# BUTSpeechFIT/TS-ASR-Whisper

Measured on AMD Instinct MI355X. Metric: train utterances/sec (30 s clips) whisper-large-v3-turbo DiCoW, higher is better.
Workload: dtype bf16; 1 GPU; whisper-large-v3-turbo DiCoW fine-tune step, per-GPU batch 16, L=128, decoder frozen, bf16 AMP; global_batch=16, parallelism=dp1, split_streams=False, trainable_params=637306880

## Files before the change

ts-asr-whisper_amd/csrc/gemm.hip:

```cpp
#include <stdlib.h>
#include "common.h"

#define BM 128
#define BN 128
#define BK 64
#define STAGE_BYTES (BM * BK * 2)
#define NT_LDS_BYTES (4 * STAGE_BYTES)
#define NT_FDDT_FLAGS (DICOW_EPI_BIAS | DICOW_EPI_RESIDUAL | DICOW_EPI_OUT_F32 | DICOW_EPI_FDDT)
#define NT_RES_FLAGS (DICOW_EPI_BIAS | DICOW_EPI_RESIDUAL | DICOW_EPI_OUT_F32)
#define NT_RES_LN_FLAGS (NT_RES_FLAGS | DICOW_EPI_LNSTAT)
#define NT_FDDT_LN_FLAGS (NT_FDDT_FLAGS | DICOW_EPI_LNSTAT)
#define NT_QKV_LN_FLAGS (DICOW_EPI_BIAS | DICOW_EPI_SCALE_N | DICOW_EPI_LNFOLD)
#define NT_FC1I_LN_FLAGS (DICOW_EPI_BIAS | DICOW_EPI_GELU | DICOW_EPI_LNFOLD)
#define NT_FC1T_LN_FLAGS (DICOW_EPI_BIAS | DICOW_EPI_GELU | DICOW_EPI_GELU_DAUX | DICOW_EPI_LNFOLD)

typedef __attribute__((address_space(3))) void lds_void_t;
typedef const __attribute__((address_space(1))) void gbl_void_t;

__device__ __forceinline__ void glds16(const void* gsrc, void* lds_dst) {
    __builtin_amdgcn_global_load_lds((gbl_void_t*)gsrc, (lds_void_t*)lds_dst, 16, 0, 0);
}

#ifndef NT_GM
#define NT_GM 8
// ... 507 lines not shown
__device__ __forceinline__ float ln_dpp(float old, float x) {
    return __int_as_float(__builtin_amdgcn_update_dpp(__float_as_int(old), __float_as_int(x), CTRL, 0xf, BANK, false));
}
template <int CTRL>
__device__ __forceinline__ float ln_merge(float a, float b, bool bit) {
    const float keep = bit ? b : a, send = bit ? a : b;
    return keep + ln_dpp<CTRL>(0.f, send);
}
__device__ __forceinline__ float ln_xor4(float x) { return ln_dpp<0x114, 0xA>(ln_dpp<0x104, 0x5>(0.f, x), x); }
__device__ __forceinline__ float ln_merge4(float a, float b, bool bit) {
    const float keep = bit ? b : a, send = bit ? a : b;
    return keep + ln_xor4(send);
}
#include "gemm_ntr.inc"
#ifndef NT2_MASK
#define NT2_MASK 0
#endif
#ifndef NT2_SLOTS
#define NT2_SLOTS 2
#endif
#ifndef NT2_DELAY
#define NT2_DELAY 0
#endif
#ifndef NTQ_MASK
#define NTQ_MASK 0
#endif
#if defined(DICOW_EXPERIMENTS) || defined(DICOW_ABLATIONS) || NT2_MASK || NTQ_MASK
#define NT_EXPERIMENT_KERNELS 1
#include "experiments/gemm_nt2.inc"
#include "experiments/gemm_ntq.inc"
#else
#define NT_EXPERIMENT_KERNELS 0
#endif

#ifdef DICOW_ABLATIONS
#include "experiments/gemm_nt256s.inc"
#endif

#include <atomic>
#include <mutex>
static std::atomic<int> g_gemm_cus{0};
extern "C" int dicow_set_gemm_cus(int n) { return g_gemm_cus.exchange(n > 0 ? n : 0); }

#include <map>
#include <mutex>
#include <string>
static std::mutex g_disp_mu;
static std::map<std::string, long> g_disp;
static void disp_note(const char* fmt, int a0 = 0, int a1 = 0, int a2 = 0) {
    char b[96];
    snprintf(b, sizeof b, fmt, a0, a1, a2);
    std::lock_guard<std::mutex> lk(g_disp_mu);
    ++g_disp[b];
}
extern "C" int dicow_gemm_dispatch_log(char* buf, int cap) {
    std::lock_guard<std::mutex> lk(g_disp_mu);
    int n = 0;
    for (const auto& kv : g_disp) {
        const int w = snprintf(buf ? buf + n : nullptr, buf && cap > n ? cap - n : 0, "%s\t%ld\n", kv.first.c_str(), kv.second);
        if (w < 0) break;
        n += w;
        if (buf && n >= cap) { n = cap - 1; break; }
    }
    return n;
}

#ifndef NT_BIG_TILES
#define NT_BIG_TILES 200
#endif
#ifndef NT64_MAX_TILES128
#define NT64_MAX_TILES128 128
#endif

#define NT_EPILOGUES_COMMON(X)                                                                                                  \
    X(0) X(DICOW_EPI_BIAS) X(DICOW_EPI_BIAS | DICOW_EPI_SCALE_N) X(DICOW_EPI_BIAS | DICOW_EPI_GELU) X(NT_RES_FLAGS)             \
    X(DICOW_EPI_BIAS | DICOW_EPI_GELU | DICOW_EPI_GELU_DAUX) X(DICOW_EPI_MUL_AUX) X(DICOW_EPI_MUL_AUX | DICOW_EPI_COLSUM)
#ifdef DICOW_EXPERIMENTS
#define NT_HAS_LN_EPILOGUES 1
#define NT_EPILOGUES_LN(BOTH, W35) W35(NT_RES_LN_FLAGS) W35(NT_FDDT_LN_FLAGS) BOTH(NT_QKV_LN_FLAGS) BOTH(NT_FC1I_LN_FLAGS) BOTH(NT_FC1T_LN_FLAGS)
#else
#define NT_HAS_LN_EPILOGUES 0
#define NT_EPILOGUES_LN(BOTH, W35)
#endif
#define NT_EPILOGUES(BOTH, W35) BOTH(-1) NT_EPILOGUES_COMMON(BOTH) W35(NT_FDDT_FLAGS) NT_EPILOGUES_LN(BOTH, W35)

static int g_ncu_all = 256;
static int nt_ncu() {
    const int lim = g_gemm_cus.load();
    return (lim > 0 && lim < g_ncu_all) ? lim : g_ncu_all;
}

static void gemm_nt_setup() {
    (void)hipFuncSetAttribute((const void*)gemm_nt_kernel<2, false>, hipFuncAttributeMaxDynamicSharedMemorySize, NT_LDS_BYTES);
    (void)hipFuncSetAttribute((const void*)gemm_nt128t_kernel, hipFuncAttributeMaxDynamicSharedMemorySize, NT_LDS_BYTES);
    (void)hipFuncSetAttribute((const void*)gemm_nt64_kernel<8>, hipFuncAttributeMaxDynamicSharedMemorySize, 8 * 16384);
    (void)hipFuncSetAttribute((const void*)gemm_nt64_kernel<4>, hipFuncAttributeMaxDynamicSharedMemorySize, 4 * 16384);
    (void)hipFuncSetAttribute((const void*)gemm_nt_kernel<2, true>, hipFuncAttributeMaxDynamicSharedMemorySize, NT_LDS_BYTES);
#define W35(F) (void)hipFuncSetAttribute((const void*)gemm_ntr_kernel<(F), 3, 5>, hipFuncAttributeMaxDynamicSharedMemorySize, NTR_LDS);
#define BOTH(F) (void)hipFuncSetAttribute((const void*)gemm_ntr_kernel<(F), 4, 4>, hipFuncAttributeMaxDynamicSharedMemorySize, NTR_LDS); W35(F)
    NT_EPILOGUES(BOTH, W35)
#undef BOTH
#undef W35
    hipDeviceProp_t pr;
    int dev = 0;
    (void)hipGetDevice(&dev);
    if (hipGetDeviceProperties(&pr, dev) == hipSuccess) g_ncu_all = pr.multiProcessorCount;
}

static int nt_ct_flags(int flags) {
    switch (flags) {
#define X(F) case (F):
        NT_EPILOGUES(X, X)
#undef X
            return flags;
        default: return -1;
    }
}
static void ntr_launch(int ct_flags, bool use35, dim3 grid, hipStream_t stream, const dicow_gemm_args& a) {
#define W35(F) case (F): hipLaunchKernelGGL((gemm_ntr_kernel<(F), 3, 5>), grid, dim3(256), NTR_LDS, stream, a); break;
#define BOTH(F) case (F):                                                                                                       \
        if (use35) hipLaunchKernelGGL((gemm_ntr_kernel<(F), 3, 5>), grid, dim3(256), NTR_LDS, stream, a);                       \
        else hipLaunchKernelGGL((gemm_ntr_kernel<(F), 4, 4>), grid, dim3(256), NTR_LDS, stream, a);                             \
        break;
    switch (ct_flags) { NT_EPILOGUES(BOTH, W35) }
#undef BOTH
#undef W35
}

enum nt_family_t {
    NT_FAM_SKINNY,
    NT_FAM_RING,
    NT_FAM_64,
    NT_FAM_128T,
    NT_FAM_GENERIC
};
struct nt_plan_t {
    nt_family_t family;
    bool off32, big;
    int grid;
    int stages64;
    bool use35;
    int colsum_rows;
    int ncu;
    bool wide_ok;
    int64_t w35, w44;
    int splitk;
};
struct nt_knobs_t { int variant, big_tiles; };

static int nt_splitk_count(const dicow_gemm_args& a, int64_t tiles128) {
    if (a.batch > 1 || (a.flags & ~DICOW_EPI_OUT_F32) != 0 || a.bias || a.residual || a.aux) return 1;
    if (a.K % BK != 0 || a.K < 8192 || a.M <= 16) return 1;
    if (tiles128 >= 2 * g_ncu_all) return 1;
    const int nk = a.K / BK;
    int best = 1;
    for (int sp = 2; sp <= 64; ++sp) {
        if (nk % sp != 0 || nk / sp < 16) continue;
        best = sp;
        if (tiles128 * sp >= 2 * g_ncu_all) break;
    }
    return best;
}

static nt_plan_t nt_plan(const dicow_gemm_args& a, int ncu, int variant = 0, int big_tiles = NT_BIG_TILES) {
    nt_plan_t p = {};
    const int batch = a.batch > 0 ? a.batch : 1;
    const int64_t tiles128 = (int64_t)dicow_cdiv(a.M, BM) * dicow_cdiv(a.N, BN);
// ... 866 lines not shown
```

ts-asr-whisper_amd/engine.py:

```python
import contextlib
import os
from types import SimpleNamespace as NS

import torch

from . import _lib as L
from . import ops

BF16, F32 = torch.bfloat16, torch.float32
CLS = ("silence_linear", "target_linear", "non_target_linear", "overlap_linear")


def _e(shape, dtype, dev):
    return torch.empty(shape, dtype=dtype, device=dev)


def _ceil(a, b):
    return (a + b - 1) // b * b


WGRAD_SIDE_STREAM = os.environ.get("DICOW_WGRAD_STREAM", "0") == "1"
WGRAD_STREAM_PRIORITY = int(os.environ.get("DICOW_WGRAD_STREAM_PRIORITY", "-1"))
_WGRAD_STREAMS = {}

# ... 12 lines not shown
SPLIT_DEC = os.environ.get("DICOW_SPLIT_DEC", "1") != "0"
SPLIT_BWD = os.environ.get("DICOW_SPLIT_BWD", "1") != "0"
SPLIT_BWD_WGRAD = os.environ.get("DICOW_SPLIT_BWD_WGRAD", "alt")
SPLIT_BWD_MEM_FRACTION = float(os.environ.get("DICOW_SPLIT_BWD_MEM_FRACTION", "0.6"))
SPLIT_IN_CAPTURE = os.environ.get("DICOW_SPLIT_IN_CAPTURE", "0") == "1"
SPLIT_FWD_PARTS = int(os.environ.get("DICOW_SPLIT_FWD_PARTS", "2"))
_FWD_STREAMS = {}


def _split_allowed():
    return SPLIT_IN_CAPTURE or not torch.cuda.is_current_stream_capturing()


def fwd_side_stream(dev, k=0):
    cur = torch.cuda.current_stream(dev)
    key = (dev.index, cur.cuda_stream, k)
    st = _FWD_STREAMS.get(key)
    if st is None:
        st = _FWD_STREAMS[key] = torch.cuda.Stream(device=dev, priority=-1)
    return st


def _fwd_parts(B, T, dev):
    n = SPLIT_FWD_PARTS if (SPLIT_FWD_PARTS > 2 and B % SPLIT_FWD_PARTS == 0) else 2
    main_st, Bp = torch.cuda.current_stream(dev), B // n
    parts = []
    for k in range(n):
        st = main_st if k == 0 else fwd_side_stream(dev, k - 1)
        if k:
            st.wait_stream(main_st)
        parts.append((st, slice(k * Bp * T, (k + 1) * Bp * T), slice(k * Bp, (k + 1) * Bp)))
    return main_st, parts, Bp


class GradSink:

    def __init__(self, params, dev, extra_rows=None):
        self.index, self.direct = {}, {}
        off = 0
        extra_rows = extra_rows or {}
        for p in params:
            if p is None or not p.requires_grad or id(p) in self.index or id(p) in self.direct:
                continue
            if getattr(p, "_direct_grad", None) is not None:
                self.direct[id(p)] = p._direct_grad
                continue
            n = p.numel() + extra_rows.get(id(p), 0)
            self.index[id(p)] = (off, p.shape, p.numel())
            off += _ceil(n, 64)
        self.flat = torch.zeros(max(off, 1), dtype=F32, device=dev)

    def get(self, p):
        if p is None:
            return None
        if id(p) in self.direct:
            return self.direct[id(p)]
        if id(p) not in self.index:
            return None
        off, shape, n = self.index[id(p)]
        return self.flat[off:off + n].view(shape)

    def result(self, p):
        return None if (p is None or id(p) in self.direct) else self.get(p)

    def is_direct(self, p):
        return p is not None and id(p) in self.direct

    def raw(self, p, n):
        if id(p) in self.direct:
            d = self.direct[id(p)]
            assert d.numel() == n, "GradSink.raw: a flat-store gradient has no padding rows"
            return d.view(-1)
        off, _, _ = self.index[id(p)]
        return self.flat[off:off + n]


class LinW:
    __slots__ = ("w", "wt", "b", "N", "K")


_BIAS_COPIES = None


def prep_linear(weights, biases, dev, need_t=True, n_pad=None, scale_info=None, bias_buf=None):
    K = weights[0].shape[1]
    Ns = [w.shape[0] for w in weights]
    N = sum(Ns)
    Np = N if n_pad is None else n_pad
    lw = LinW()
    lw.N, lw.K = Np, K
    lw.w = torch.zeros(Np, K, dtype=BF16, device=dev) if Np != N else _e((Np, K), BF16, dev)
    lw.wt = (torch.zeros(K, Np, dtype=BF16, device=dev) if Np != N else _e((K, Np), BF16, dev)) if need_t else None
    off = 0
    for w, n in zip(weights, Ns):
        ops.cast_transpose_bf16(w.detach(), out=lw.w[off:off + n], out_t=None if lw.wt is None else lw.wt[:, off:off + n],
                                ld=K, ld_t=Np)
        off += n
    if biases is None or all(b is None for b in biases):
        lw.b = None
    else:
        if bias_buf is not None and _BIAS_COPIES is not None and len(Ns) > 1:
            off = 0
            for b, n in zip(biases, Ns):
                if b is not None:
                    _BIAS_COPIES.append((bias_buf[off:off + n], b.detach()))
                off += n
            lw.b = bias_buf
        else:
            parts = [(b.detach() if b is not None else torch.zeros(n, dtype=F32, device=dev)) for b, n in zip(biases, Ns)]
            lw.b = parts[0] if len(parts) == 1 else torch.cat(parts)
    return lw


def prep_attention(att, dev, fuse_qkv=True, bias_buf=None):
    a = NS()
    if fuse_qkv:
        a.qkv = prep_linear([att.q_proj.weight, att.k_proj.weight, att.v_proj.weight],
                            [att.q_proj.bias, None, att.v_proj.bias], dev, bias_buf=bias_buf)
    else:
        a.q = prep_linear([att.q_proj.weight], [att.q_proj.bias], dev)
        a.kv = prep_linear([att.k_proj.weight, att.v_proj.weight], [None, att.v_proj.bias], dev)
    a.o = prep_linear([att.out_proj.weight], [att.out_proj.bias], dev)
    return a


def fddt_ptrs(fddt, cfg):
    if fddt is None:
        return ops.MODE_NONE, (None,) * 4, (None,) * 4
    w, b = [], []
    for c in CLS:
        m = getattr(fddt, c, None)
        if fddt.bias_only:
            w.append(None)
            b.append(None if m is None else m)
        else:
            w.append(None if m is None else m.weight)
            b.append(None if m is None else m.bias)
    return (ops.MODE_BIAS if fddt.bias_only else ops.MODE_DIAG), tuple(w), tuple(b)


def fddt_is_full(fddt):
    return fddt is not None and not fddt.is_diagonal


def prep_full_fddt(fddt, dev):
    D = fddt.d_model
    w = NS(use=0)
    w.Wc = torch.zeros(4 * D, D, dtype=BF16, device=dev)
    w.Wct = torch.zeros(D, 4 * D, dtype=BF16, device=dev)
    w.bias = torch.zeros(4 * D, dtype=F32, device=dev)
    for c, name in enumerate(CLS):
        m = getattr(fddt, name, None)
        if m is not None:
            w.use |= 1 << c
            ops.cast_transpose_bf16(m.weight.detach(), out=w.Wc[c * D:(c + 1) * D], out_t=w.Wct[:, c * D:(c + 1) * D], ld=D, ld_t=4 * D)
            w.bias[c * D:(c + 1) * D] = m.bias.detach()
    return w


def full_fddt_fwd(w, h, stno, bstride, rows, T, D):
    hb = h if h.dtype == BF16 else ops.cast_bf16(h)
    y4 = _e((rows, 4 * D), BF16, h.device)
    ops.gemm_nt(hb, w.Wc, y4, rows, 4 * D, D, bias=w.bias)
    out = _e((rows, D), F32, h.device)
    L.call("dicow_fddt_full_combine_fwd", y4.data_ptr(), h.data_ptr(), int(h.dtype == BF16), stno.data_ptr(), bstride, w.use,
           out.data_ptr(), rows, T, D, L.stream())
    return out, hb


def full_fddt_bwd(fddt, w, hb, g, stno, bstride, G, rows, T, D):
    dev = g.device
    d_y4 = torch.zeros(rows, 4 * D, dtype=BF16, device=dev)
    gh = _e((rows, D), F32, dev)
    L.call("dicow_fddt_full_combine_bwd", g.data_ptr(), stno.data_ptr(), bstride, w.use, d_y4.data_ptr(), gh.data_ptr(), rows, T, D,
           L.stream())
    ops.gemm_nt(d_y4, w.Wct, gh, rows, D, 4 * D, flags=L.EPI_ACCUM)
    for c, name in enumerate(CLS):
        m = getattr(fddt, name, None)
        if m is None:
            continue
        sl = d_y4[:, c * D:(c + 1) * D]
        if G.get(m.bias) is not None:
            ops.colsum_bf16(sl, G.get(m.bias))
        if G.get(m.weight) is not None:
            ops.gemm_tn(sl, hb, G.get(m.weight), rows, D, D, lda=4 * D, ldb=D, ldc=D)
    return gh


QK_LOG2 = os.environ.get("DICOW_QK_LOG2", "1") != "0"
FUSE_NEXT_FDDT = True
LN_FOLD = os.environ.get("DICOW_LN_FOLD", "0") == "1"
Q_SCALE = 0.125 * (ops.LOG2E if QK_LOG2 else 1.0)


def linear_fwd(x, lw, M, out_dtype=BF16, residual=None, gelu_aux=None, flags=0, scale=1.0, scale_ncols=0, out=None, fddt=None):
    dev = x.device
    if out is None:
        out = _e((M, lw.N), out_dtype, dev)
    ops.gemm_nt(x, lw.w, out, M, lw.N, lw.K, bias=lw.b, residual=residual, aux=gelu_aux,
                flags=flags | ((L.EPI_GELU | L.EPI_GELU_DAUX) if gelu_aux is not None else 0), scale=scale, scale_ncols=scale_ncols, fddt=fddt)
    return out


def linear_dgrad(dy, lw, M, aux=None, out=None, out_dtype=BF16, accumulate=False, dy_cols=None, colsum_out=None):
# ... 769 lines not shown
        for i in range(nl - 1, lo - 1, -1):
            lyr, w, Ls = enc.layers[i], W.layers[i], S.layers[i]
            att, ln, ln2 = lyr.self_attn, lyr.self_attn_layer_norm, lyr.final_layer_norm
            fd = enc.fddts[i] if (cfg.use_fddt and i < len(enc.fddts)) else None
            mode, fw, fb = fddt_ptrs(fd, cfg)
            prev_b2 = enc.layers[i - 1].fc2.bias if i > 0 else None
            d_u, d_xln2 = _e((rows, F_), BF16, dev), _e((rows, D), BF16, dev)
            g2, g2b, d_o = _e((rows, D), F32, dev), _e((rows, D), BF16, dev), _e((rows, D), BF16, dev)
            d_qkv, d_xln = _e((rows, 3 * D), BF16, dev), _e((rows, D), BF16, dev)
            g0, g0b = _e((rows, D), F32, dev), (_e((rows, D), BF16, dev) if i > 0 else None)
            keep += [d_u, d_xln2, g2, g2b, d_o, d_qkv, d_xln, g0, g0b, g, gb]
            qkv = Ls.qkv
            evs = []
            for k, (st_, r, bsl) in enumerate(parts):
                gg = G.get if k == 0 else shget
                with torch.cuda.stream(st_):
                    linear_dgrad(gb[r], w.fc2, rh, aux=Ls.u[r], colsum_out=gg(lyr.fc1.bias), out=d_u[r])
                    linear_dgrad(d_u[r], w.fc1, rh, out=d_xln2[r])
                    ops.fddt_ln_bwd(Ls.h2[r], rh, D, mode=ops.MODE_NONE, ln_w=ln2.weight.detach(), mean=Ls.mean2[r], rstd=Ls.rstd2[r],
                                    d_y=d_xln2[r], g_res=g[r], g_out=g2[r], g_out_bf16=g2b[r], dln_w=gg(ln2.weight), dln_b=gg(ln2.bias),
                                    colsum_out=gg(att.out_proj.bias))
                    linear_dgrad(g2b[r], w.att.o, rh, out=d_o[r])
                    delta = _e((2, Bh, H, T), F32, dev)
                    ops.attn_bwd(heads(qkv[r][:, :D], Bh, T, H), heads(qkv[r][:, D:2 * D], Bh, T, H), heads(qkv[r][:, 2 * D:], Bh, T, H),
                                 heads(Ls.o[r], Bh, T, H), heads(d_o[r], Bh, T, H), Ls.lse[bsl], delta, heads(d_qkv[r][:, :D], Bh, T, H),
                                 heads(d_qkv[r][:, D:2 * D], Bh, T, H), heads(d_qkv[r][:, 2 * D:], Bh, T, H), dq_scale=0.125, q_log2=QK_LOG2,
                                 dq_colsum=gg(att.q_proj.bias), dv_colsum=gg(att.v_proj.bias))
                    linear_dgrad(d_qkv[r], w.att.qkv, rh, out=d_xln[r])
                    ops.fddt_ln_bwd(Ls.h_in[r], rh, D, mode=mode, stno=S.stno[bsl.start * sstep:], stno_bstride=Ls.bstride, T=T, w=fw, b=fb,
                                    ln_w=ln.weight.detach(), mean=Ls.mean[r], rstd=Ls.rstd[r], d_y=d_xln[r], g_res=g2[r], g_out=g0[r],
                                    g_out_bf16=g0b[r] if g0b is not None else None, dln_w=gg(ln.weight), dln_b=gg(ln.bias),
                                    dw=tuple(gg(x) for x in fw), db=tuple(gg(x) for x in fb), colsum_out=gg(prev_b2))
                    keep.append(delta)
                    evs.append(st_.record_event())
            tg = ops.TnGroup()
            linear_wgrad(gb, Ls.a, G.get(lyr.fc2.weight), rows, group=tg, param=lyr.fc2.weight)
            linear_wgrad(d_u, Ls.xln2, G.get(lyr.fc1.weight), rows, group=tg, param=lyr.fc1.weight)
            linear_wgrad(g2b, Ls.o, G.get(att.out_proj.weight), rows, group=tg, param=att.out_proj.weight)
            qkv_wgrad(d_qkv, Ls.xln, G.get(att.q_proj.weight), G.get(att.k_proj.weight), G.get(att.v_proj.weight), rows, D, group=tg,
                      params=(att.q_proj.weight, att.k_proj.weight, att.v_proj.weight))
            if pending is not None:
                finish(pending)
            pending = (i, tg, evs[0], evs[1])
            g, gb = g0, g0b
        finish(pending)
        while deferred:
            settle(deferred.pop(0))
        main_st.wait_stream(side_st)
        if third_st is not None:
            main_st.wait_stream(third_st)
        if lo > 0:
            pb = enc.layers[lo - 1].fc2.bias
            if G.get(pb) is not None:
                G.get(pb).add_(sh.view[id(pb)])
        del keep
        return g, gb

    def _stem_backward(self, S, g, G):
        enc, cfg, W = self.enc, self.cfg, self.W
        dev = g.device
        T, D = S.T, cfg.d_model
        B, Tin, M = S.B0, 2 * T, cfg.num_mel_bins
        rows = B * T
        gpos = G.get(enc.embed_positions.weight)
        if gpos is not None:
            ops.sum_over_batch(g.view(B, T * D), gpos)
        conv_train = enc.conv1.weight.requires_grad or enc.conv2.weight.requires_grad or enc.conv1.bias.requires_grad
        init_fddt = enc.initial_fddt if (cfg.use_fddt and cfg.use_pre_pos_fddt) else None
        mode, fw, fb = fddt_ptrs(init_fddt, cfg)
        dw = tuple(G.get(x) for x in fw)
        db = tuple(G.get(x) for x in fb)
        if not conv_train and all(x is None for x in dw + db):
            return
        if W.full_init is not None:
            d_x2 = ops.cast_bf16(full_fddt_bwd(init_fddt, W.full_init, S.x2b, g, S.stno, 4 * T, G, rows, T, D))
        else:
            d_x2 = _e((rows, D), BF16, dev)
            ops.fddt_ln_bwd(S.x2, rows, D, mode=mode, stno=S.stno, T=T, w=fw, b=fb, g_res=g, g_out_bf16=d_x2, dw=dw, db=db)
        if not conv_train:
            return
        conv_stem_bwd(enc, W, S.stem, d_x2, G)


class DecoderEngine:
    def __init__(self, model):
        self.model = model
        self.cfg = model.config

    def prepare(self):
        dec, cfg = self.model.model.decoder, self.cfg
        dev = dec.embed_tokens.weight.device
        W = NS(layers=[])
        for lyr in dec.layers:
            w = NS()
            w.sa = prep_attention(lyr.self_attn, dev)
            w.ca = prep_attention(lyr.encoder_attn, dev, fuse_qkv=False)
            w.fc1 = prep_linear([lyr.fc1.weight], [lyr.fc1.bias], dev)
            w.fc2 = prep_linear([lyr.fc2.weight], [lyr.fc2.bias], dev)
            sa, ca = lyr.self_attn, lyr.encoder_attn
            w.lora = NS(sa_qkv=prep_lora([sa.q_proj, sa.k_proj, sa.v_proj], dev), sa_o=prep_lora([sa.out_proj], dev),
                        ca_q=prep_lora([ca.q_proj], dev), ca_kv=prep_lora([ca.k_proj, ca.v_proj], dev), ca_o=prep_lora([ca.out_proj], dev),
                        fc1=prep_lora([lyr.fc1], dev), fc2=prep_lora([lyr.fc2], dev))
            W.layers.append(w)
        W.vpad = _ceil(cfg.vocab_size, 128)
        W.head = prep_linear([self.model.proj_out.weight], None, dev, n_pad=W.vpad)
        self.W = W
        return W

    def refresh_adapters(self):
        with ops.cast_group():
            for w in self.W.layers:
                for la in vars(w.lora).values():
                    if la is not None:
                        la.refresh()

    def _layers_fwd(self, enc_bf, B, T, Lq, h):
        model, cfg, W = self.model, self.cfg, self.W
        dec = model.model.decoder
        dev = enc_bf.device
        D, H, F_ = cfg.d_model, cfg.decoder_attention_heads, cfg.decoder_ffn_dim
        rows = B * Lq
        out = []
        for i, lyr in enumerate(dec.layers):
            w = W.layers[i]
            la = w.lora
            Ls = NS(h_in=h)
            ln = lyr.self_attn_layer_norm
            Ls.x1, Ls.m1, Ls.r1 = _e((rows, D), BF16, dev), _e((rows,), F32, dev), _e((rows,), F32, dev)
            ops.fddt_ln_fwd(h, rows, D, ln_w=ln.weight.detach(), ln_b=ln.bias.detach(), y_bf16=Ls.x1, mean=Ls.m1, rstd=Ls.r1)
            Ls.qkv = linear_fwd(Ls.x1, w.sa.qkv, rows, flags=L.EPI_SCALE_N, scale=Q_SCALE, scale_ncols=D)
            Ls.t_qkv = lora_fwd(Ls.x1, la.sa_qkv, Ls.qkv, rows, q_scale=Q_SCALE)
            Ls.o1, Ls.lse1 = _e((rows, D), BF16, dev), _e((B, H, Lq), F32, dev)
            ops.attn_fwd(heads(Ls.qkv[:, :D], B, Lq, H), heads(Ls.qkv[:, D:2 * D], B, Lq, H), heads(Ls.qkv[:, 2 * D:], B, Lq, H),
                         heads(Ls.o1, B, Lq, H), Ls.lse1, causal=True, q_log2=QK_LOG2)
            Ls.h2 = linear_fwd(Ls.o1, w.sa.o, rows, out_dtype=F32, residual=h)
            Ls.t_o1 = lora_fwd(Ls.o1, la.sa_o, Ls.h2, rows)
            ln = lyr.encoder_attn_layer_norm
            Ls.x2, Ls.m2, Ls.r2 = _e((rows, D), BF16, dev), _e((rows,), F32, dev), _e((rows,), F32, dev)
            ops.fddt_ln_fwd(Ls.h2, rows, D, ln_w=ln.weight.detach(), ln_b=ln.bias.detach(), y_bf16=Ls.x2, mean=Ls.m2, rstd=Ls.r2)
            Ls.q = linear_fwd(Ls.x2, w.ca.q, rows, flags=L.EPI_SCALE_N, scale=Q_SCALE, scale_ncols=D)
            Ls.t_q = lora_fwd(Ls.x2, la.ca_q, Ls.q, rows, q_scale=Q_SCALE)
            Ls.kv = linear_fwd(enc_bf, w.ca.kv, B * T)
            Ls.t_kv = lora_fwd(enc_bf, la.ca_kv, Ls.kv, B * T)
            Ls.o2, Ls.lse2 = _e((rows, D), BF16, dev), _e((B, H, Lq), F32, dev)
            ops.attn_fwd(heads(Ls.q, B, Lq, H), heads(Ls.kv[:, :D], B, T, H), heads(Ls.kv[:, D:], B, T, H), heads(Ls.o2, B, Lq, H),
                         Ls.lse2, q_log2=QK_LOG2)
            Ls.h3 = linear_fwd(Ls.o2, w.ca.o, rows, out_dtype=F32, residual=Ls.h2)
            Ls.t_o2 = lora_fwd(Ls.o2, la.ca_o, Ls.h3, rows)
            ln = lyr.final_layer_norm
            Ls.x3, Ls.m3, Ls.r3 = _e((rows, D), BF16, dev), _e((rows,), F32, dev), _e((rows,), F32, dev)
            ops.fddt_ln_fwd(Ls.h3, rows, D, ln_w=ln.weight.detach(), ln_b=ln.bias.detach(), y_bf16=Ls.x3, mean=Ls.m3, rstd=Ls.r3)
            Ls.u = _e((rows, F_), BF16, dev)
            if la.fc1 is None:
                Ls.a, Ls.t_fc1 = linear_fwd(Ls.x3, w.fc1, rows, gelu_aux=Ls.u), None
            else:
                Ls.a = linear_fwd(Ls.x3, w.fc1, rows)
                Ls.t_fc1 = lora_fwd(Ls.x3, la.fc1, Ls.a, rows, gelu=True, gelu_aux=Ls.u)
            h = linear_fwd(Ls.a, w.fc2, rows, out_dtype=F32, residual=Ls.h3)
            Ls.t_fc2 = lora_fwd(Ls.a, la.fc2, h, rows)
            out.append(Ls)
        return h, out

    def forward(self, enc_bf, B, T, decoder_input_ids, labels, upp_labels, ts=None):
        model, cfg, W = self.model, self.cfg, self.W
        dec = model.model.decoder
        dev = enc_bf.device
        D, H, F_ = cfg.d_model, cfg.decoder_attention_heads, cfg.decoder_ffn_dim
        Lq = decoder_input_ids.shape[1]
        if Lq > cfg.max_target_positions:
            raise ValueError(f"decoder length {Lq} exceeds max_target_positions {cfg.max_target_positions}")
        rows = B * Lq
        S = NS(B=B, T=T, Lq=Lq, ids=decoder_input_ids.contiguous(), enc_bf=enc_bf)
        h = _e((rows, D), F32, dev)
        ops.embed_fwd(S.ids, dec.embed_tokens.weight.detach(), dec.embed_positions.weight.detach(), h)
        S.xf, S.mf, S.rf = _e((rows, D), BF16, dev), _e((rows,), F32, dev), _e((rows,), F32, dev)
        split = (SPLIT_FWD and SPLIT_DEC and B % 2 == 0 and B * T >= SPLIT_FWD_MIN_ROWS and enc_bf.is_cuda
                 and _split_allowed() and not model.proj_out.weight.requires_grad
                 and not any(p.requires_grad for p in dec.parameters()))
        if split:
            main_st, parts, Bh = _fwd_parts(B, 1, dev)
        else:
            main_st, parts, Bh = None, ((None, slice(0, B), slice(0, B)),), B
        S.parts = []
        for st_, _, bsl in parts:
            rq, re = slice(bsl.start * Lq, bsl.stop * Lq), slice(bsl.start * T, bsl.stop * T)
            with (torch.cuda.stream(st_) if st_ is not None else contextlib.nullcontext()):
                hl, layers = self._layers_fwd(enc_bf[re], Bh, T, Lq, h[rq])
                ops.fddt_ln_fwd(hl, Bh * Lq, D, ln_w=dec.layer_norm.weight.detach(), ln_b=dec.layer_norm.bias.detach(), y_bf16=S.xf[rq],
                                mean=S.mf[rq], rstd=S.rf[rq])
            S.parts.append(NS(st=st_, rq=rq, re=re, B=Bh, h_last=hl, layers=layers))
        for st_, _, _ in parts[1:]:
            main_st.wait_stream(st_)
        logits = _e((rows, W.vpad), BF16, dev)
        ops.gemm_nt(S.xf, W.head.w, logits, rows, W.vpad, D)
        S.logits = logits
        loss = None
        if labels is not None:
            S.labels = labels.contiguous().view(-1)
            S.upp = None if upp_labels is None else upp_labels.contiguous().view(-1)
            S.lse, S.row_loss = _e((rows,), F32, dev), _e((rows,), F32, dev)
            S.choice = _e((rows,), torch.int32, dev)
            S.acc = torch.zeros(2, dtype=F32, device=dev)
            S.soft = ts is not None
            S.ce = ops.ce_args(logits, W.vpad, rows, cfg.vocab_size, S.labels, S.upp, S.soft, ts, S.lse, S.row_loss, S.choice,
                               S.acc[0:1], S.acc[1:2])
            ops.ce_loss_fwd(S.ce)
            if S.soft:
                S.denom = S.acc[1].clamp(min=1.0)
            else:
                S.denom = torch.full((), float(rows), dtype=F32, device=dev)
            loss = S.acc[0] / S.denom
        return loss, logits.view(B, Lq, W.vpad)[:, :, :cfg.vocab_size], S

    def _layers_bwd(self, layers, enc_bf, B, T, Lq, g, gb, G, d_enc):
        model, cfg, W = self.model, self.cfg, self.W
        dec = model.model.decoder
        dev = g.device
        D, H, F_ = cfg.d_model, cfg.decoder_attention_heads, cfg.decoder_ffn_dim
        rows = B * Lq
        nl = len(dec.layers)
        for i in range(nl - 1, -1, -1):
            lyr, w, Ls = dec.layers[i], W.layers[i], layers[i]
            la = w.lora
            linear_wgrad(gb, Ls.a, G.get(lyr.fc2.weight), rows)
            if la.fc2 is None:
                d_u = linear_dgrad(gb, w.fc2, rows, aux=Ls.u)
            else:
                d_u = _e((rows, F_), BF16, dev)
                lora_bwd(gb, Ls.a, Ls.t_fc2, la.fc2, rows, G, dx=linear_dgrad(gb, w.fc2, rows, out_dtype=F32), mul_aux=Ls.u, dx_out=d_u)
            bias_grad(d_u, G.get(lyr.fc1.bias))
            linear_wgrad(d_u, Ls.x3, G.get(lyr.fc1.weight), rows)
            d_x3 = linear_dgrad(d_u, w.fc1, rows)
            lora_bwd(d_u, Ls.x3, Ls.t_fc1, la.fc1, rows, G, dx=d_x3)
            g3, g3b = _e((rows, D), F32, dev), _e((rows, D), BF16, dev)
            ln = lyr.final_layer_norm
            ops.fddt_ln_bwd(Ls.h3, rows, D, ln_w=ln.weight.detach(), mean=Ls.m3, rstd=Ls.r3, d_y=d_x3, g_res=g, g_out=g3,
                            g_out_bf16=g3b, dln_w=G.get(ln.weight), dln_b=G.get(ln.bias),
                            colsum_out=G.get(lyr.encoder_attn.out_proj.bias))
            att = lyr.encoder_attn
            linear_wgrad(g3b, Ls.o2, G.get(att.out_proj.weight), rows)
            d_o2 = linear_dgrad(g3b, w.ca.o, rows)
            lora_bwd(g3b, Ls.o2, Ls.t_o2, la.ca_o, rows, G, dx=d_o2)
            dq = _e((rows, D), BF16, dev)
            dkv = _e((B * T, 2 * D), BF16, dev)
            delta = _e((2, B, H, Lq), F32, dev)
            ops.attn_bwd(heads(Ls.q, B, Lq, H), heads(Ls.kv[:, :D], B, T, H), heads(Ls.kv[:, D:], B, T, H), heads(Ls.o2, B, Lq, H),
                         heads(d_o2, B, Lq, H), Ls.lse2, delta, heads(dq, B, Lq, H), heads(dkv[:, :D], B, T, H),
                         heads(dkv[:, D:], B, T, H), dq_scale=0.125, q_log2=QK_LOG2)
            bias_grad(dq, G.get(att.q_proj.bias))
            bias_grad(dkv[:, D:], G.get(att.v_proj.bias))
            linear_wgrad(dq, Ls.x2, G.get(att.q_proj.weight), rows)
            linear_wgrad(dkv[:, :D], enc_bf, G.get(att.k_proj.weight), B * T)
            linear_wgrad(dkv[:, D:], enc_bf, G.get(att.v_proj.weight), B * T)
            if d_enc is not None:
                linear_dgrad(dkv, w.ca.kv, B * T, out=d_enc, accumulate=True)
            lora_bwd(dkv, enc_bf, Ls.t_kv, la.ca_kv, B * T, G, dx=d_enc)
            d_x2 = linear_dgrad(dq, w.ca.q, rows)
            lora_bwd(dq, Ls.x2, Ls.t_q, la.ca_q, rows, G, dx=d_x2)
            g2, g2b = _e((rows, D), F32, dev), _e((rows, D), BF16, dev)
            ln = lyr.encoder_attn_layer_norm
            ops.fddt_ln_bwd(Ls.h2, rows, D, ln_w=ln.weight.detach(), mean=Ls.m2, rstd=Ls.r2, d_y=d_x2, g_res=g3, g_out=g2,
                            g_out_bf16=g2b, dln_w=G.get(ln.weight), dln_b=G.get(ln.bias),
                            colsum_out=G.get(lyr.self_attn.out_proj.bias))
            att = lyr.self_attn
            linear_wgrad(g2b, Ls.o1, G.get(att.out_proj.weight), rows)
            d_o1 = linear_dgrad(g2b, w.sa.o, rows)
            lora_bwd(g2b, Ls.o1, Ls.t_o1, la.sa_o, rows, G, dx=d_o1)
            d_qkv = _e((rows, 3 * D), BF16, dev)
            qkv = Ls.qkv
            ops.attn_bwd(heads(qkv[:, :D], B, Lq, H), heads(qkv[:, D:2 * D], B, Lq, H), heads(qkv[:, 2 * D:], B, Lq, H),
                         heads(Ls.o1, B, Lq, H), heads(d_o1, B, Lq, H), Ls.lse1, delta, heads(d_qkv[:, :D], B, Lq, H),
                         heads(d_qkv[:, D:2 * D], B, Lq, H), heads(d_qkv[:, 2 * D:], B, Lq, H), causal=True, dq_scale=0.125, q_log2=QK_LOG2)
            bias_grad(d_qkv[:, :D], G.get(att.q_proj.bias))
            bias_grad(d_qkv[:, 2 * D:], G.get(att.v_proj.bias))
            linear_wgrad(d_qkv[:, :D], Ls.x1, G.get(att.q_proj.weight), rows)
            linear_wgrad(d_qkv[:, D:2 * D], Ls.x1, G.get(att.k_proj.weight), rows)
            linear_wgrad(d_qkv[:, 2 * D:], Ls.x1, G.get(att.v_proj.weight), rows)
            d_x1 = linear_dgrad(d_qkv, w.sa.qkv, rows)
            lora_bwd(d_qkv, Ls.x1, Ls.t_qkv, la.sa_qkv, rows, G, dx=d_x1)
            g1, g1b = _e((rows, D), F32, dev), _e((rows, D), BF16, dev)
            ln = lyr.self_attn_layer_norm
            ops.fddt_ln_bwd(Ls.h_in, rows, D, ln_w=ln.weight.detach(), mean=Ls.m1, rstd=Ls.r1, d_y=d_x1, g_res=g2, g_out=g1,
                            g_out_bf16=g1b, dln_w=G.get(ln.weight), dln_b=G.get(ln.bias),
                            colsum_out=G.get(dec.layers[i - 1].fc2.bias) if i > 0 else None)
            g, gb = g1, g1b
        return g

    def backward(self, S, grad_loss, G, need_d_enc=True, d_logits_ext=None):
        model, cfg, W = self.model, self.cfg, self.W
        dec = model.model.decoder
        dev = S.logits.device
        D, H, F_ = cfg.d_model, cfg.decoder_attention_heads, cfg.decoder_ffn_dim
        B, T, Lq = S.B, S.T, S.Lq
        rows = B * Lq
        d_logits = _e((rows, W.vpad), BF16, dev)
        scale = (grad_loss.to(F32) / S.denom).reshape(1)
        S.ce.d_logits = d_logits.data_ptr()
        ops.ce_loss_bwd(S.ce, scale)
        ge = G.get(model.proj_out.weight)
        if ge is not None:
            if G.is_direct(model.proj_out.weight) and W.vpad != cfg.vocab_size:
                tmp = torch.zeros(W.vpad, D, dtype=F32, device=dev)
                ops.gemm_tn(d_logits, S.xf, tmp, rows, W.vpad, D)
                ge.add_(tmp[:cfg.vocab_size])
            else:
                ops.gemm_tn(d_logits, S.xf, G.raw(model.proj_out.weight, W.vpad * D).view(W.vpad, D), rows, W.vpad, D)
        d_xf = linear_dgrad(d_logits, W.head, rows)
        g = _e((rows, D), F32, dev)
        nl = len(dec.layers)
        d_enc = torch.zeros(B * T, D, dtype=F32, device=dev) if need_d_enc else None
        split = len(S.parts) > 1
        if split:
            main_st = torch.cuda.current_stream(dev)
            for P in S.parts[1:]:
                P.st.wait_stream(main_st)
        for P in S.parts:
            rq, re, rows_p = P.rq, P.re, P.B * Lq
            with (torch.cuda.stream(P.st) if split else contextlib.nullcontext()):
                gb = _e((rows_p, D), BF16, dev)
                ops.fddt_ln_bwd(P.h_last, rows_p, D, ln_w=dec.layer_norm.weight.detach(), mean=S.mf[rq], rstd=S.rf[rq], d_y=d_xf[rq], g_out=g[rq],
                                g_out_bf16=gb, dln_w=G.get(dec.layer_norm.weight), dln_b=G.get(dec.layer_norm.bias),
                                colsum_out=G.get(dec.layers[nl - 1].fc2.bias))
                g_emb = self._layers_bwd(P.layers, S.enc_bf[re], P.B, T, Lq, g[rq], gb, G, d_enc[re] if need_d_enc else None)
        if split:
            for P in S.parts[1:]:
                main_st.wait_stream(P.st)
        gt, gp = G.get(dec.embed_tokens.weight), G.get(dec.embed_positions.weight)
        if gt is not None or gp is not None:
            assert not split
            ops.embed_bwd(S.ids, g_emb, gt, gp, D)
        return d_enc


class CtcEngine:

    def __init__(self, enc):
        self.enc = enc
        self.cfg = enc.config

    def prepare(self):
        enc, cfg = self.enc, self.cfg
        dev = enc.lm_head.weight.device
        D = cfg.d_model
        W = NS()
        W.att = prep_attention(enc.additional_self_attention_layer, dev) if hasattr(enc, "additional_self_attention_layer") else None
        W.lyr = None
        if hasattr(enc, "additional_layer"):
            lyr = enc.additional_layer
            W.lyr = NS(att=prep_attention(lyr.self_attn, dev), fc1=prep_linear([lyr.fc1.weight], [lyr.fc1.bias], dev),
                       fc2=prep_linear([lyr.fc2.weight], [lyr.fc2.bias], dev))
            W.att = None
        if hasattr(enc, "subsample_conv1"):
            W.c1, W.c1_t = ops.conv_weight_pack(enc.subsample_conv1.weight.detach(), 3 * D, want_t=True)
            W.c2, W.c2_t = ops.conv_weight_pack(enc.subsample_conv2.weight.detach(), 3 * D, want_t=True)
        W.cpad = _ceil(cfg.vocab_size + 1, 128)
        W.head = prep_linear([enc.lm_head.weight], None, dev, n_pad=W.cpad)
        self.W = W
        return W

    def frames(self, T):
        return T // 4 if hasattr(self.enc, "subsample_conv1") else T

    def forward(self, enc_bf, B, T, labels, enc_f32=None):
        cfg, W = self.cfg, self.W
        dev = enc_bf.device
        S = self.encode_logits(enc_bf, B, T, enc_f32)
        logits, Tn = S.logits, S.Tn
        Cc = cfg.vocab_size + 1
        lab = labels.contiguous()
        Lc = lab.shape[1]
        S.lse, S.nll, S.tlen = _e((B * Tn,), F32, dev), _e((B,), F32, dev), _e((B,), F32, dev)
        Smax = 2 * Lc + 1
        S.ab = _e((2, B, Tn, Smax), F32, dev)
        S.acc = torch.zeros(1, dtype=F32, device=dev)
        S.labels = lab
        S.ctc = ops.ctc_args(logits, W.cpad, B, Tn, Cc, lab, S.lse, S.ab[0], S.ab[1], S.nll, S.tlen, S.acc)
        ops.ctc_loss_fwd(S.ctc)
        if cfg.ctc_loss_reduction != "mean":
            raise L.DicowError("only ctc_loss_reduction='mean' (reference default) is implemented")
        return S.acc[0] / B, S

    def encode_logits(self, enc_bf, B, T, enc_f32=None, out=None):
        enc, cfg, W = self.enc, self.cfg, self.W
        dev = enc_bf.device
        D, H = cfg.d_model, cfg.encoder_attention_heads
        rows = B * T
        S = NS(B=B, T=T, enc_bf=enc_bf)
        sub = hasattr(enc, "subsample_conv1")
        if sub and T % 4 != 0:
            raise L.DicowError("pre_ctc_sub_sample needs max_source_positions % 4 == 0")
        h = enc_bf
        hpad = None
        if W.lyr is not None:
            hf, S.lyr = plain_layer_fwd(enc.additional_layer, W.lyr, enc_f32 if enc_f32 is not None else enc_bf.float(), B, T, H,
                                        cfg.encoder_ffn_dim)
            h = ops.cast_bf16(hf)
            if sub:
                hpad = torch.zeros(B, T + 2, D, dtype=BF16, device=dev)
                hpad[:, 1:T + 1].copy_(h.view(B, T, D))
        elif W.att is not None:
            S.qkv = linear_fwd(enc_bf, W.att.qkv, rows, flags=L.EPI_SCALE_N, scale=Q_SCALE, scale_ncols=D)
            S.o, S.lse_a = _e((rows, D), BF16, dev), _e((B, H, T), F32, dev)
            ops.attn_fwd(heads(S.qkv[:, :D], B, T, H), heads(S.qkv[:, D:2 * D], B, T, H), heads(S.qkv[:, 2 * D:], B, T, H),
                         heads(S.o, B, T, H), S.lse_a, q_log2=QK_LOG2)
            if sub:
                hpad = _e((B, T + 2, D), BF16, dev)
# ... 95 lines not shown
```

Baseline: 119.5 utt/s.

## Batch decoder cross-attention dK/dV dgrads into one concatenated GEMM

Instead of issuing one small accumulating dgrad GEMM per decoder layer into d_enc, per-layer dK/dV gradients are written into a single wide buffer and the cross-attention K/V transposed weights are packed contiguously. One long-K GEMM then produces d_enc directly in f32, which also removes the zero-init of d_enc. The aim is to cut launch count and repeated read-modify-write of the f32 d_enc, at the cost of a larger temporary buffer (B*T x nl*2D bf16) and deferring LoRA backward to after the loop.

```diff
diff --git a/ts-asr-whisper_amd/csrc/gemm.hip b/ts-asr-whisper_amd/csrc/gemm.hip
--- a/ts-asr-whisper_amd/csrc/gemm.hip
+++ b/ts-asr-whisper_amd/csrc/gemm.hip
@@ -613,7 +613,7 @@
 #define NT_HAS_LN_EPILOGUES 0
 #define NT_EPILOGUES_LN(BOTH, W35)
 #endif
-#define NT_EPILOGUES(BOTH, W35) BOTH(-1) NT_EPILOGUES_COMMON(BOTH) W35(NT_FDDT_FLAGS) NT_EPILOGUES_LN(BOTH, W35)
+#define NT_EPILOGUES(BOTH, W35) BOTH(-1) NT_EPILOGUES_COMMON(BOTH) W35(NT_FDDT_FLAGS) NT_EPILOGUES_LN(BOTH, W35) BOTH(DICOW_EPI_OUT_F32)
 
 static int g_ncu_all = 256;
 static int nt_ncu() {
diff --git a/ts-asr-whisper_amd/engine.py b/ts-asr-whisper_amd/engine.py
--- a/ts-asr-whisper_amd/engine.py
+++ b/ts-asr-whisper_amd/engine.py
@@ -118,7 +118,7 @@
 _BIAS_COPIES = None
 
 
-def prep_linear(weights, biases, dev, need_t=True, n_pad=None, scale_info=None, bias_buf=None):
+def prep_linear(weights, biases, dev, need_t=True, n_pad=None, scale_info=None, bias_buf=None, wt_out=None):
     K = weights[0].shape[1]
     Ns = [w.shape[0] for w in weights]
     N = sum(Ns)
@@ -126,11 +126,15 @@
     lw = LinW()
     lw.N, lw.K = Np, K
     lw.w = torch.zeros(Np, K, dtype=BF16, device=dev) if Np != N else _e((Np, K), BF16, dev)
-    lw.wt = (torch.zeros(K, Np, dtype=BF16, device=dev) if Np != N else _e((K, Np), BF16, dev)) if need_t else None
+    if wt_out is not None:
+        assert need_t and Np == N and tuple(wt_out.shape) == (K, N) and wt_out.dtype == BF16 and wt_out.stride(1) == 1
+        lw.wt = wt_out
+    else:
+        lw.wt = (torch.zeros(K, Np, dtype=BF16, device=dev) if Np != N else _e((K, Np), BF16, dev)) if need_t else None
     off = 0
     for w, n in zip(weights, Ns):
         ops.cast_transpose_bf16(w.detach(), out=lw.w[off:off + n], out_t=None if lw.wt is None else lw.wt[:, off:off + n],
-                                ld=K, ld_t=Np)
+                                ld=K, ld_t=Np if lw.wt is None else lw.wt.stride(0))
         off += n
     if biases is None or all(b is None for b in biases):
         lw.b = None
@@ -148,14 +152,14 @@
     return lw
 
 
-def prep_attention(att, dev, fuse_qkv=True, bias_buf=None):
+def prep_attention(att, dev, fuse_qkv=True, bias_buf=None, kv_wt_out=None):
     a = NS()
     if fuse_qkv:
         a.qkv = prep_linear([att.q_proj.weight, att.k_proj.weight, att.v_proj.weight],
                             [att.q_proj.bias, None, att.v_proj.bias], dev, bias_buf=bias_buf)
     else:
         a.q = prep_linear([att.q_proj.weight], [att.q_proj.bias], dev)
-        a.kv = prep_linear([att.k_proj.weight, att.v_proj.weight], [None, att.v_proj.bias], dev)
+        a.kv = prep_linear([att.k_proj.weight, att.v_proj.weight], [None, att.v_proj.bias], dev, wt_out=kv_wt_out)
     a.o = prep_linear([att.out_proj.weight], [att.out_proj.bias], dev)
     return a
 
@@ -1091,6 +1095,9 @@
         conv_stem_bwd(enc, W, S.stem, d_x2, G)
 
 
+DEC_DENC_CONCAT = True
+
+
 class DecoderEngine:
     def __init__(self, model):
         self.model = model
@@ -1100,10 +1107,12 @@
         dec, cfg = self.model.model.decoder, self.cfg
         dev = dec.embed_tokens.weight.device
         W = NS(layers=[])
-        for lyr in dec.layers:
+        nl, D = len(dec.layers), cfg.d_model
+        W.ca_kv_wt = _e((D, nl * 2 * D), BF16, dev)
+        for i, lyr in enumerate(dec.layers):
             w = NS()
             w.sa = prep_attention(lyr.self_attn, dev)
-            w.ca = prep_attention(lyr.encoder_attn, dev, fuse_qkv=False)
+            w.ca = prep_attention(lyr.encoder_attn, dev, fuse_qkv=False, kv_wt_out=W.ca_kv_wt[:, (nl - 1 - i) * 2 * D:(nl - i) * 2 * D])
             w.fc1 = prep_linear([lyr.fc1.weight], [lyr.fc1.bias], dev)
             w.fc2 = prep_linear([lyr.fc2.weight], [lyr.fc2.bias], dev)
             sa, ca = lyr.self_attn, lyr.encoder_attn
@@ -1221,13 +1230,14 @@
             loss = S.acc[0] / S.denom
         return loss, logits.view(B, Lq, W.vpad)[:, :, :cfg.vocab_size], S
 
-    def _layers_bwd(self, layers, enc_bf, B, T, Lq, g, gb, G, d_enc):
+    def _layers_bwd(self, layers, enc_bf, B, T, Lq, g, gb, G, d_enc, concat=False):
         model, cfg, W = self.model, self.cfg, self.W
         dec = model.model.decoder
         dev = g.device
         D, H, F_ = cfg.d_model, cfg.decoder_attention_heads, cfg.decoder_ffn_dim
         rows = B * Lq
         nl = len(dec.layers)
+        dkv_all = _e((B * T, nl * 2 * D), BF16, dev) if concat else None
         for i in range(nl - 1, -1, -1):
             lyr, w, Ls = dec.layers[i], W.layers[i], layers[i]
             la = w.lora
@@ -1251,7 +1261,7 @@
             d_o2 = linear_dgrad(g3b, w.ca.o, rows)
             lora_bwd(g3b, Ls.o2, Ls.t_o2, la.ca_o, rows, G, dx=d_o2)
             dq = _e((rows, D), BF16, dev)
-            dkv = _e((B * T, 2 * D), BF16, dev)
+            dkv = dkv_all[:, (nl - 1 - i) * 2 * D:(nl - i) * 2 * D] if concat else _e((B * T, 2 * D), BF16, dev)
             delta = _e((2, B, H, Lq), F32, dev)
             ops.attn_bwd(heads(Ls.q, B, Lq, H), heads(Ls.kv[:, :D], B, T, H), heads(Ls.kv[:, D:], B, T, H), heads(Ls.o2, B, Lq, H),
                          heads(d_o2, B, Lq, H), Ls.lse2, delta, heads(dq, B, Lq, H), heads(dkv[:, :D], B, T, H),
@@ -1261,9 +1271,10 @@
             linear_wgrad(dq, Ls.x2, G.get(att.q_proj.weight), rows)
             linear_wgrad(dkv[:, :D], enc_bf, G.get(att.k_proj.weight), B * T)
             linear_wgrad(dkv[:, D:], enc_bf, G.get(att.v_proj.weight), B * T)
-            if d_enc is not None:
+            if d_enc is not None and not concat:
                 linear_dgrad(dkv, w.ca.kv, B * T, out=d_enc, accumulate=True)
-            lora_bwd(dkv, enc_bf, Ls.t_kv, la.ca_kv, B * T, G, dx=d_enc)
+            if not concat:
+                lora_bwd(dkv, enc_bf, Ls.t_kv, la.ca_kv, B * T, G, dx=d_enc)
             d_x2 = linear_dgrad(dq, w.ca.q, rows)
             lora_bwd(dq, Ls.x2, Ls.t_q, la.ca_q, rows, G, dx=d_x2)
             g2, g2b = _e((rows, D), F32, dev), _e((rows, D), BF16, dev)
@@ -1293,6 +1304,10 @@
                             g_out_bf16=g1b, dln_w=G.get(ln.weight), dln_b=G.get(ln.bias),
                             colsum_out=G.get(dec.layers[i - 1].fc2.bias) if i > 0 else None)
             g, gb = g1, g1b
+        if concat:
+            ops.gemm_nt(dkv_all, W.ca_kv_wt, d_enc, B * T, D, nl * 2 * D, lda=dkv_all.stride(0), ldb=W.ca_kv_wt.stride(0), ldc=d_enc.stride(0))
+            for i in range(nl - 1, -1, -1):
+                lora_bwd(dkv_all[:, (nl - 1 - i) * 2 * D:(nl - i) * 2 * D], enc_bf, layers[i].t_kv, W.layers[i].lora.ca_kv, B * T, G, dx=d_enc)
         return g
 
     def backward(self, S, grad_loss, G, need_d_enc=True, d_logits_ext=None):
@@ -1317,7 +1332,8 @@
         d_xf = linear_dgrad(d_logits, W.head, rows)
         g = _e((rows, D), F32, dev)
         nl = len(dec.layers)
-        d_enc = torch.zeros(B * T, D, dtype=F32, device=dev) if need_d_enc else None
+        concat = DEC_DENC_CONCAT and need_d_enc
+        d_enc = (_e((B * T, D), F32, dev) if concat else torch.zeros(B * T, D, dtype=F32, device=dev)) if need_d_enc else None
         split = len(S.parts) > 1
         if split:
             main_st = torch.cuda.current_stream(dev)
@@ -1330,7 +1346,7 @@
                 ops.fddt_ln_bwd(P.h_last, rows_p, D, ln_w=dec.layer_norm.weight.detach(), mean=S.mf[rq], rstd=S.rf[rq], d_y=d_xf[rq], g_out=g[rq],
                                 g_out_bf16=gb, dln_w=G.get(dec.layer_norm.weight), dln_b=G.get(dec.layer_norm.bias),
                                 colsum_out=G.get(dec.layers[nl - 1].fc2.bias))
-                g_emb = self._layers_bwd(P.layers, S.enc_bf[re], P.B, T, Lq, g[rq], gb, G, d_enc[re] if need_d_enc else None)
+                g_emb = self._layers_bwd(P.layers, S.enc_bf[re], P.B, T, Lq, g[rq], gb, G, d_enc[re] if need_d_enc else None, concat=concat)
         if split:
             for P in S.parts[1:]:
                 main_st.wait_stream(P.st)
```

Result: faster. 122.9 utt/s (median of 6 runs) (+2.9%).
